# markkurossi/mpc

Hardware: AMD Instinct MI355X
Metric: AND-gates/sec (garble+eval), AES-128 circuit batch (higher is better)
Workload: dtype u32 (AES T-table / 128-bit label XOR, integer); 1 GPU; aes_128.circ 36663 gates / 6400 AND, batch=1024 instances per GPU, 32-byte garbling key; instances_per_gpu=1024, levels=308, launches_per_garble=1, schedule=fused-flat, hash_phases=89, lds_live_labels=1053, graph=True, outputs_ok=True, device_memory=gc_dev_alloc / gc_dev_upload (C ABI); no torch in the process, gathers=0

## Files before the change

### include/gcengine.h

```cpp
#ifndef GCENGINE_H
#define GCENGINE_H

#include <stddef.h>
#include <stdint.h>

#ifdef __cplusplus
extern "C" {
#endif

typedef struct gc_label { uint64_t d0, d1; } gc_label;
typedef struct gc_wire { gc_label l0, l1; } gc_wire;
typedef struct gc_gate {
    uint32_t in0, in1, out;
    uint8_t op;
    uint8_t pad_[3];
    uint32_t level;
} gc_gate;

enum {
    GC_XOR = 0, GC_XNOR = 1, GC_AND = 2, GC_OR = 3, GC_INV = 4
};

enum {
    GC_OK = 0,
// ... 23 lines not shown
    uint32_t n_xor, n_xnor, n_and, n_or, n_inv;
    uint32_t nslots;
    uint32_t n_steps;
    uint32_t n_hash_phases;
    uint32_t n_fused_steps;
    uint32_t n_lds_slots;
    uint32_t n_flat_slots;
    uint32_t n_flat_outs;
    uint32_t n_flat_terms;
    uint32_t n_flat_steps;
    uint32_t n_flat_units;
} gc_plan_info;

gc_plan *gc_plan_create(const gc_gate *gates, uint32_t ngates, uint32_t nwires, uint32_t ninputs,
                        uint32_t noutputs, int *status);
gc_plan *gc_plan_create_chain(const gc_gate *const *gates, const uint32_t *ngates, const uint32_t *nwires, const uint32_t *nin,
                              const uint32_t *nout, const uint32_t *const *wiring, uint32_t nsteps, int *status);
void gc_plan_free(gc_plan *);
int gc_plan_get_info(const gc_plan *, gc_plan_info *out);
int gc_plan_simulate(const gc_plan *, const uint8_t *in_bits, uint8_t *out_bits);
int gc_plan_describe(const gc_plan *, uint32_t *level_of_gate, uint32_t *tweak_of_gate,
                     uint32_t *row_of_gate, uint32_t *slot_of_gate);
int gc_plan_fingerprint(const gc_plan *, uint64_t *fp);

typedef struct gc_ctx gc_ctx;
typedef struct gc_circ gc_circ;

int gc_device_count(void);
gc_ctx *gc_ctx_create(int device, int *status);
void gc_ctx_destroy(gc_ctx *);
int gc_ctx_sync(gc_ctx *);
int gc_ctx_coop_stats(gc_ctx *, int *state, uint64_t *timeouts);
int gc_ctx_pci_bus_id(gc_ctx *, char *buf, size_t len);
void *gc_ctx_stream(gc_ctx *);

typedef struct gc_graph gc_graph;
int gc_ctx_capture_begin(gc_ctx *);
int gc_ctx_capture_end(gc_ctx *, gc_graph **out);
int gc_graph_launch(gc_graph *);
void gc_graph_free(gc_graph *);

gc_circ *gc_circ_load(gc_ctx *, const gc_gate *gates, uint32_t ngates, uint32_t nwires,
                      uint32_t ninputs, uint32_t noutputs, int *status);
void gc_circ_free(gc_circ *);
const gc_plan *gc_circ_plan(const gc_circ *);
int gc_circ_set_schedule(gc_circ *, int schedule);
// ... 313 lines not shown
```

### mpc_amd/csrc/aes_device.h

```cpp
#pragma once

#include <hip/hip_runtime.h>

#include <cstdint>

namespace gc {

constexpr int kTeWords = 4 * 256;

__device__ __forceinline__ uint32_t rotr32(uint32_t v, uint32_t n) { return __builtin_amdgcn_alignbit(v, v, n); }

__device__ __forceinline__ void load_te_tables(uint32_t *te, const uint32_t *__restrict__ g_te0) {
    for (uint32_t i = threadIdx.x; i < 256; i += blockDim.x) {
        uint32_t t = g_te0[i];
        te[i] = t;
        te[256 + i] = rotr32(t, 8);
        te[512 + i] = rotr32(t, 16);
        te[768 + i] = rotr32(t, 24);
    }
}

template <int NR, int N>
__device__ __forceinline__ void aes_encrypt_n(uint32_t (&s)[N][4], const uint32_t *__restrict__ rk,
                                              const uint32_t *te) {
// ... 78 lines not shown
        s[k][0] = GC_LAST(a0, a1, a2, a3) ^ rk[4 * NR + 0];
        s[k][1] = GC_LAST(a1, a2, a3, a0) ^ rk[4 * NR + 1];
        s[k][2] = GC_LAST(a2, a3, a0, a1) ^ rk[4 * NR + 2];
        s[k][3] = GC_LAST(a3, a0, a1, a2) ^ rk[4 * NR + 3];
#undef GC_LAST
#undef GC_SB
    }
}

constexpr int kTeDualBytes = 256 * 256;

__device__ __forceinline__ void te_dual_check(const uint32_t *te);

__device__ __forceinline__ void load_te_dual(uint32_t *te, const uint32_t *__restrict__ g_te0) {
    te_dual_check(te);
    const uint32_t c = threadIdx.x & 31;
    for (uint32_t x = threadIdx.x >> 5; x < 256; x += blockDim.x >> 5) {
        const uint32_t t = g_te0[x];
        te[x * 64 + c] = t;
        te[x * 64 + 32 + c] = rotr32(t, 16);
    }
}

#define GC_PERM_SEL(k) (0x0c0c0000u | ((4u + (k)) << 8))

using lds_u32 = __attribute__((address_space(3))) const uint32_t;

__device__ __forceinline__ void te_dual_check(const uint32_t *te) {
    if ((uint32_t)(uintptr_t)te != 0u) __builtin_trap();
}

__device__ __forceinline__ uint32_t te_dual(uint32_t word, uint32_t sel, uint32_t lane_off) {
    const uint32_t addr = __builtin_amdgcn_perm(word, lane_off, sel);
    return *(lds_u32 *)(uintptr_t)addr;
}

__device__ __forceinline__ uint32_t xor3(uint32_t a, uint32_t b, uint32_t c) {
    return __builtin_amdgcn_bitop3_b32(a, b, c, 0x96);
}

__device__ __forceinline__ void te_round_addrs(const uint32_t (&a)[4], uint32_t lo0, uint32_t lo2, uint32_t (&ad)[16]) {
    const uint32_t sel0 = GC_PERM_SEL(0), sel1 = GC_PERM_SEL(1), sel2 = GC_PERM_SEL(2), sel3 = GC_PERM_SEL(3);
#pragma unroll
    for (int c = 0; c < 4; c++) {
        ad[4 * c + 0] = __builtin_amdgcn_perm(a[c], lo0, sel3);
        ad[4 * c + 1] = __builtin_amdgcn_perm(a[(c + 2) & 3], lo2, sel1);
// ... 136 lines not shown
            __builtin_amdgcn_sched_barrier(0);
#pragma unroll
            for (int k = 0; k < N; k++)
#pragma unroll
                for (int i = 0; i < 16; i++) t[k][i] = *(lds_u32 *)(uintptr_t)ad[k][i];
            __builtin_amdgcn_sched_barrier(0);
            te_final_combine<NR, N, FEED>(t, rk, fin, s);
        }
    }
}

template <int NR>
__device__ __forceinline__ void load_round_keys(uint32_t (&rk)[4 * (NR + 1)], const uint32_t *__restrict__ g_rk) {
#pragma unroll
    for (int i = 0; i < 4 * (NR + 1); i++) rk[i] = __builtin_amdgcn_readfirstlane(g_rk[i]);
}

template <int NR, int NS>
__device__ __forceinline__ void load_round_keys_split(uint32_t (&rk)[4 * (NR + 1)], const uint32_t *__restrict__ g_rk,
                                                      uint32_t vz) {
#pragma unroll
    for (int i = 0; i < 4 * (NR + 1); i++)
        rk[i] = i < NS ? (uint32_t)__builtin_amdgcn_readfirstlane(g_rk[i]) : g_rk[i + vz];
}

template <int NR, int N>
__device__ __forceinline__ void hash_dual_n(const uint32_t (&k)[N][4], uint4 (&out)[N],
                                            const uint32_t (&rk)[4 * (NR + 1)], const uint32_t *te, uint32_t lo0) {
    uint32_t s[N][4];
#pragma unroll
    for (int i = 0; i < N; i++) {
        s[i][0] = k[i][0];
        s[i][1] = k[i][1];
        s[i][2] = k[i][2];
        s[i][3] = k[i][3];
    }
    aes_encrypt_dual<NR, N, 1>(s, rk, te, lo0);
#pragma unroll
    for (int i = 0; i < N; i++) out[i] = make_uint4(s[i][1], s[i][0], s[i][3], s[i][2]);
}

template <int NR>
__device__ __forceinline__ uint4 hash_dual(const uint32_t (&k)[4], const uint32_t (&rk)[4 * (NR + 1)],
                                           const uint32_t *te, uint32_t lo0) {
    uint32_t s[1][4] = {{k[0], k[1], k[2], k[3]}};
    aes_encrypt_dual<NR, 1, 1>(s, rk, te, lo0);
// ... 143 lines not shown
```

### mpc_amd/csrc/engine.cpp

```cpp
#include "engine.h"

#include <algorithm>
#include <atomic>
#include <chrono>
#include <cstdlib>
#include <cstdio>
#include <cstring>
#include <new>
#include <stdexcept>

namespace gc {

thread_local char tls_error[512] = "";

void set_error(const char *what, hipError_t e) {
    std::snprintf(tls_error, sizeof tls_error, "%s: %s (%d)", what, hipGetErrorString(e), (int)e);
    (void)hipGetLastError();
}

int on_exception() noexcept {
    try {
        throw;
    } catch (const std::bad_alloc &) {
        std::snprintf(tls_error, sizeof tls_error, "host allocation failed (std::bad_alloc)");
// ... 775 lines not shown
static int run_levels(gc_batch *b, bool eval, const uint4 *T, const uint4 *rnd = nullptr) {
    hipStream_t s = b->circ->ctx->stream;
    const Plan &p = b->circ->plan.p;
    if (b->schedule == 1 && b->g.lds_wires && want_flat(b)) {
        FusedFlatArgs f{};
        f.prog = b->circ->d_fl_prog;
        f.units = b->circ->d_fl_units;
        f.hgslot = b->circ->d_fl_hgslot;
        f.ogslot = b->circ->d_fl_ogslot;
        f.in_lds = b->circ->d_fl_in_lds;
        f.nunits = (uint32_t)p.fl_units.size();
        f.ninputs = p.info.ninputs;
        f.nls = p.n_flat_slots;
        f.ustride = p.fl_unit_stride;
        f.W = b->d_W;
        f.R = b->d_R;
        f.T = const_cast<uint4 *>(T);
        f.rk = b->d_rk;
        f.te0 = b->circ->ctx->d_te0;
        f.rounds = b->rounds;
        f.prof = b->d_prof;
        f.rnd = rnd;
        f.has_or = p.info.n_or != 0;
        GC_HIP(launch_fused_flat(eval, f, b->g, s));
        b->last_launches = f.nunits ? 1 : 0;
        b->have_all_wires = false;
        return GC_OK;
    }
    if (b->schedule == 1 && b->g.lds_wires) {
        FusedLdsArgs f{};
        f.descs = b->circ->d_fdescs;
        f.gslot = b->circ->d_fgslot;
        f.steps = b->circ->d_fsteps;
        f.in_lds = b->circ->d_in_lds;
        f.nsteps = (uint32_t)p.fsteps.size();
        f.chunks = b->circ->d_fchunks;
        f.nchunks = (uint32_t)p.fchunks.size();
        f.ninputs = p.info.ninputs;
        f.nls = p.n_lds_slots;
        f.W = b->d_W;
        f.R = b->d_R;
        f.T = const_cast<uint4 *>(T);
        f.rk = b->d_rk;
        f.te0 = b->circ->ctx->d_te0;
        f.rounds = b->rounds;
        f.store_all = b->store_all;
// ... 659 lines not shown
}
bool gc_circ_flat_job(gc_circ *c, gc::FlatJob *j, size_t *lds_bytes, bool *has_or) {
    if (!c || !j) return false;
    circ_ensure_flat(c);
    const Plan &p = c->plan.p;
    if (p.n_flat_slots == 0xffffffffu || p.fl_units.empty() || p.info.slab_rows >= (1u << 22) || !c->d_fl_prog) return false;
    const size_t need = fused_flat_bytes(p.n_flat_slots, 0, p.fl_unit_stride);
    if (need > (size_t)160 * 1024) return false;
    *j = FlatJob{};
    j->prog = (const uint4 *)c->d_fl_prog;
    j->units = c->d_fl_units;
    j->hgslot = c->d_fl_hgslot;
    j->ogslot = c->d_fl_ogslot;
    j->in_lds = c->d_fl_in_lds;
    j->nunits = (uint32_t)p.fl_units.size();
    j->ninputs = p.info.ninputs;
    j->ti_log2 = 0;
    j->zslot = p.n_flat_slots - 1;
    j->ustride = p.fl_unit_stride;
    j->w_tile = p.info.nslots;
    j->t_tile = std::max<uint32_t>(p.info.slab_rows, 1);
    j->te0 = c->ctx->d_te0;
    j->batch = 1;
    if (lds_bytes) *lds_bytes = need;
    if (has_or) *has_or = p.info.n_or != 0;
    return true;
}

void gc_circ_release_batch(gc_circ *c, gc_batch *b) {
    if (c && b) pool_put(c, b);
}

int gc_pass_dev(gc_circ *c, bool eval, const uint8_t *key, size_t keylen, const gc_label *r, const void *d_store,
                const uint32_t *d_in_idx, const uint32_t *d_out_idx, const gc_label *slab_host, size_t slab_rows,
                gc_batch **bout, const gc::StoreXchg *d_xchg) {
    if (!c || !bout || !d_store || (!eval && !r)) return GC_E_ARG;
    gc_batch *b = *bout;
    *bout = nullptr;
    const Plan &p = c->plan.p;
    if (b && (b->circ != c || b->g.batch != 1)) return GC_E_ARG;
    if (eval && (slab_rows != p.info.slab_rows || (!slab_host && slab_rows && !b))) {
        if (b) pool_put(c, b);
        return GC_E_ROWS;
    }
    int rc = GC_OK;
    if (!b) b = pool_get(c, 1, &rc);
// ... 234 lines not shown
```

### mpc_amd/csrc/fused_flat_kernels.hip

```cpp
#include "aes_device.h"
#include "kernels.h"

namespace gc {

namespace {

constexpr int TF = 1024;

constexpr int DPP_XOR1 = 0xB1;
constexpr int DPP_XOR2 = 0x4E;
constexpr int DPP_XOR3 = 0x1B;
constexpr int DPP_BC0 = 0x00;
constexpr int DPP_BC2 = 0xAA;
constexpr int DPP_PAIR0 = 0xA0;

template <int CTRL>
__device__ __forceinline__ uint32_t dpp32(uint32_t v) {
    return (uint32_t)__builtin_amdgcn_mov_dpp((int)v, CTRL, 0xf, 0xf, true);
}
template <int CTRL>
__device__ __forceinline__ uint4 dpp128(uint4 v) {
    return make_uint4(dpp32<CTRL>(v.x), dpp32<CTRL>(v.y), dpp32<CTRL>(v.z), dpp32<CTRL>(v.w));
}

// ... 320 lines not shown
    const uint64_t *q = (const uint64_t *)p;
    const uint64_t lo = __hip_atomic_load(q, __ATOMIC_RELAXED, __HIP_MEMORY_SCOPE_AGENT);
    const uint64_t hi = __hip_atomic_load(q + 1, __ATOMIC_RELAXED, __HIP_MEMORY_SCOPE_AGENT);
    return make_uint4((uint32_t)lo, (uint32_t)(lo >> 32), (uint32_t)hi, (uint32_t)(hi >> 32));
}
__device__ __forceinline__ void store_put(uint4 *p, const uint4 &v) {
    uint64_t *q = (uint64_t *)p;
    __hip_atomic_store(q, (uint64_t)v.x | ((uint64_t)v.y << 32), __ATOMIC_RELAXED, __HIP_MEMORY_SCOPE_AGENT);
    __hip_atomic_store(q + 1, (uint64_t)v.z | ((uint64_t)v.w << 32), __ATOMIC_RELAXED, __HIP_MEMORY_SCOPE_AGENT);
}

constexpr uint32_t kDepSpins = 1u << 22;
__device__ __forceinline__ uint32_t fresh_u32(const uint32_t *p) { return __hip_atomic_load(p, __ATOMIC_RELAXED, __HIP_MEMORY_SCOPE_AGENT); }
__device__ __forceinline__ void df_wait_reached(const uint32_t *p, uint32_t want, uint32_t *host_err) {
    for (uint32_t spins = 0; (int32_t)(__hip_atomic_load(p, __ATOMIC_RELAXED, __HIP_MEMORY_SCOPE_AGENT) - want) < 0;) {
        __builtin_amdgcn_s_sleep(8);
        if (++spins > kDepSpins) {
            if (host_err) __hip_atomic_fetch_max(host_err, 3u, __ATOMIC_RELAXED, __HIP_MEMORY_SCOPE_SYSTEM);
            break;
        }
    }
}

#define GC_FL_PROLOGUE(LOAD_R)                                                                               \
    const uint32_t tile = MULTI ? 0u : blockIdx.x;                                                           \
    extern __shared__ uint4 smem[];                                                                          \
    uint32_t *te = (uint32_t *)smem;                                                                         \
    const uint32_t ti_log2 = a.ti_log2, TI = 1u << ti_log2, tim = TI - 1;                                    \
    uint4 *stage = smem + kStageOff;                                                                         \
    const uint32_t ustride = a.ustride;                                                                      \
    uint4 *rl = smem + kStageOff + 2 * ustride;                                                              \
    uint4 *wl = rl + TI;                                                                                     \
     \
    const bool first_job = !MULTI || a.pad2_ == 0;                                                           \
    if (first_job) load_te_dual(te, a.te0);                                                                  \
    uint32_t rkr[4 * (NR + 1)];                                                                              \
    uint32_t vz;                                                                                             \
    asm volatile("v_mov_b32 %0, 0" : "=v"(vz));                                                              \
    load_round_keys_split<NR, (4 * (NR + 1) > 32 ? 4 * (NR + 1) - 32 : 4 * (NR + 1))>(rkr, a.rk, vz);        \
    fold_last_round_key<NR>(rkr);               \
    if (first_job && threadIdx.x < 4 * (NR + 1)) {  \
        uint32_t kv = a.rk[threadIdx.x];                                                                     \
        if (threadIdx.x >= 4 * NR) kv ^= a.rk[threadIdx.x - 4 * NR];                                         \
        ((uint32_t *)smem)[kKeyTab / 4 + threadIdx.x] = kv;                                                  \
    }                                                                                                        \
    uint4 *Wt = a.W + (size_t)tile * a.w_tile;                                                               \
    if (threadIdx.x < TI) wl[(a.zslot << ti_log2) + threadIdx.x] = make_uint4(0, 0, 0, 0);                   \
    if (LOAD_R && a.rnd) {                                                                                   \
         \
         \
        for (uint32_t i = threadIdx.x; i < ((a.ninputs + 1) << ti_log2); i += TF) {                          \
            const uint32_t j = i >> ti_log2, inst = i & tim, gi = tile * TI + inst;                          \
            uint4 v = make_uint4(0, 0, 0, 0);                                                                \
            if (gi < a.batch) {                                                                              \
                const uint4 raw = a.rnd[(size_t)gi * (a.ninputs + 1) + j];                                   \
                v = make_uint4(__builtin_bswap32(raw.y), __builtin_bswap32(raw.x), __builtin_bswap32(raw.w), \
                               __builtin_bswap32(raw.z));                                                    \
            }                                                                                                \
            if (j == 0) {                                                                                    \
                v.y |= 0x80000000u;                                                        \
                rl[inst] = v;                                                                                \
                a.Rout[(size_t)tile * TI + inst] = v;                                                        \
            } else {                                                                                         \
                const uint32_t ls = a.in_lds[j - 1];                                                         \
                Wt[((j - 1) << ti_log2) + inst] = v;                                                         \
                if (ls != 0xffffu) wl[(ls << ti_log2) + inst] = v;                                           \
            }                                                                                                \
        }                                                                                                    \
    } else {                                                                                                 \
        if (LOAD_R && threadIdx.x < TI) rl[threadIdx.x] = a.R[(size_t)tile * TI + threadIdx.x];              \
        for (uint32_t i = threadIdx.x; i < (a.ninputs << ti_log2); i += TF) {                                \
            const uint32_t w = i >> ti_log2, ls = a.in_lds[w];                                               \
            if constexpr (MULTI) {            \
                const DfBlock *dfb = LOAD_R ? (const DfBlock *)a.prof : nullptr;  \
                const uint32_t sidx = dfb ? fresh_u32(a.in_idx + w) : a.in_idx[w];                           \
                if (dfb) df_wait_reached(dfb->ver + sidx, fresh_u32((const uint32_t *)(dfb + 1) + w), dfb->host_err); \
                const uint4 v = store_get(a.store + sidx);                                                   \
                Wt[i] = v;                                                                                   \
                if (ls != 0xffffu) wl[(ls << ti_log2) + (i & tim)] = v;                                      \
                if (dfb) {  \
                    asm volatile("s_waitcnt vmcnt(0)" ::: "memory");                                         \
                    __hip_atomic_fetch_add(dfb->rd + sidx, 1u, __ATOMIC_RELAXED, __HIP_MEMORY_SCOPE_AGENT);  \
                }                                                                                            \
            } else if (ls != 0xffffu) {                                                                      \
                wl[(ls << ti_log2) + (i & tim)] = Wt[i];                                                     \
            }                                                                                                \
        }                                                                                                    \
    }                                                                                                        \
    FUnit u = uniform_unit(load_unit(a.units, 0, vz));                                             \
     \
     \
    FUnit un = load_unit(a.units, 1, vz);                                                          \
    if (threadIdx.x < u.n16) stage[threadIdx.x] = a.prog[u.off16 + threadIdx.x];                             \
     \
     \
    uint4 pre_cur = a.prog[un.off16 + threadIdx.x];                                                          \
    __syncthreads();                                                                                         \
    const uint32_t lo = te_lane_off();                                                                       \
    const uint32_t wave_base = __builtin_amdgcn_readfirstlane(threadIdx.x & ~63u);                           \
    uint64_t pacc[8] = {0, 0, 0, 0, 0, 0, 0, 0}, plast = 0;                                                  \
    if constexpr (PROF) plast = __builtin_amdgcn_s_memtime();

}

template <int NR, bool PROF, bool HAS_OR, bool MULTI>
__device__ __forceinline__ void garble_flat_body(const FlArgs &a) {
    GC_FL_PROLOGUE(true)
    uint4 *Tt = a.T + (size_t)tile * a.t_tile;
    for (uint32_t ui = 0; ui < a.nunits; ui++) {
        const uint4 *buf = stage + (ui & 1u) * ustride;
        const uint32_t nh = u.n_and + u.n_or + u.n_inv;
        GC_FPROF(0)
        const uint32_t e_hash = hlanes<2, 2, 1>(u, ti_log2);
        if (nh && u.n_or == 0 && e_hash <= kNarrowLanes) {
            garble_hash_narrow<NR, PROF>(buf, u, a, ti_log2, tim, wl, rl, Tt, Wt, lo, HashSplit{0, e_hash, 0}, pacc, &plast);
        } else if (nh) {
            const HashSplit hs = split_hash_lanes(e_hash, u.n_or != 0, kTailMaxGarble);
            const uint32_t e_all = hs.wide_end;
        for (uint32_t t0 = 0; t0 + wave_base < e_all; t0 += TF) {
// ... 380 lines not shown
hipError_t launch_fused_flat(bool eval, const FusedFlatArgs &f, const BatchGeom &g, hipStream_t s) {
    FlArgs a{};
    a.prog = (const uint4 *)f.prog;
    a.units = f.units;
    a.hgslot = f.hgslot;
    a.ogslot = f.ogslot;
    a.in_lds = f.in_lds;
    a.nunits = f.nunits;
    a.ninputs = f.ninputs;
    a.ti_log2 = g.ti_log2;
    a.zslot = f.nls - 1;
    a.ustride = f.ustride;
    a.w_tile = g.lw.tile_stride;
    a.t_tile = g.lt.tile_stride;
    a.W = f.W;
    a.R = f.R;
    a.T = f.T;
    a.rk = f.rk;
    a.te0 = f.te0;
    a.prof = f.prof;
    a.rnd = eval ? nullptr : f.rnd;
    a.Rout = const_cast<uint4 *>(f.R);
    a.batch = g.batch;
    if (a.nunits == 0) return hipSuccess;
    const size_t lds = fused_flat_bytes(f.nls, g.ti_log2, f.ustride);
#define GC_M3(KERN, NR)                                                                      \
    (f.prof ? (f.has_or ? launch_fl(KERN<NR, true, true>, a, g.ntiles, lds, s)               \
                        : launch_fl(KERN<NR, true, false>, a, g.ntiles, lds, s))             \
            : f.has_or ? launch_fl(KERN<NR, false, true>, a, g.ntiles, lds, s)              \
                       : launch_fl(KERN<NR, false, false>, a, g.ntiles, lds, s))
#define GC_M2(KERN) (f.rounds == 10 ? GC_M3(KERN, 10) : f.rounds == 12 ? GC_M3(KERN, 12) : GC_M3(KERN, 14))
    return eval ? GC_M2(k_eval_flat) : GC_M2(k_garble_flat);
#undef GC_M2
#undef GC_M3
}

template <typename K>
static hipError_t launch_jobs(K kern, const FlatJob *jobs, const uint32_t *first, uint32_t *sync, uint32_t nunits, size_t lds,
                              hipStream_t s) {
    hipError_t e = hipFuncSetAttribute((const void *)kern, hipFuncAttributeMaxDynamicSharedMemorySize, (int)lds);
    if (e != hipSuccess) return e;
    hipLaunchKernelGGL(kern, dim3(nunits), dim3(TF), lds, s, jobs, first, sync);
    return hipGetLastError();
}

template <typename K>
// ... 36 lines not shown
```

### mpc_amd/csrc/kernels.h

```cpp
#pragma once

#include <hip/hip_runtime.h>

#include <cstdint>

#include "co_multi_table.h"
#include "co_table.h"
#include "p256.h"
#include "plan.h"
#include "vole_mod.h"

namespace gc {

struct Layout {
    uint32_t ti_log2;
    uint32_t ti_mask;
    size_t row_stride;
    size_t tile_stride;
#if defined(__HIPCC__)
    __host__ __device__
#endif
    size_t at(size_t row, uint32_t inst) const {
        return (size_t)(inst >> ti_log2) * tile_stride + row * row_stride + (inst & ti_mask);
    }
// ... 83 lines not shown
    int rounds;
    bool store_all;
    uint64_t *prof;
};
size_t fused_lds_bytes(uint32_t nls, uint32_t ti_log2);
hipError_t launch_fused_lds(bool eval, const FusedLdsArgs &a, const BatchGeom &g, hipStream_t s);

struct FusedFlatArgs {
    const uint32_t *prog;
    const FUnit *units;
    const uint32_t *hgslot, *ogslot;
    const uint16_t *in_lds;
    uint32_t nunits, ninputs, nls;
    uint32_t ustride;
    uint4 *W;
    const uint4 *R;
    uint4 *T;
    const uint32_t *rk;
    const uint32_t *te0;
    int rounds;
    uint64_t *prof;
    const uint4 *rnd;
    bool has_or;
};
size_t fused_flat_bytes(uint32_t nls, uint32_t ti_log2, uint32_t ustride);
hipError_t launch_fused_flat(bool eval, const FusedFlatArgs &a, const BatchGeom &g, hipStream_t s);

struct FlatJob {
    const uint4 *prog;
    const FUnit *units;
    const uint32_t *hgslot, *ogslot;
    const uint16_t *in_lds;
    uint32_t nunits, ninputs, ti_log2, zslot;
    uint32_t ustride;
    size_t w_tile, t_tile;
    uint4 *W;
    const uint4 *R;
    uint4 *T;
    const uint32_t *rk;
    const uint32_t *te0;
    uint64_t *prof;
    const uint4 *rnd;
    uint4 *Rout;
    uint32_t batch;
    uint32_t pad_;
    uint4 *store;
    const uint32_t *in_idx;
    const uint32_t *out_slots;
    const uint32_t *out_idx;
    uint32_t nout, pad2_;
};
constexpr uint32_t kSyncHead = 4;
struct DfBlock {
    uint32_t *ver, *rd;
    uint32_t *host_err;
    uint32_t nin, nout;
    uint32_t pad_[2];
};
static_assert(sizeof(DfBlock) == 40 || sizeof(DfBlock) == 48, "DfBlock layout");
constexpr uint32_t kPoolRing = 8192;
constexpr uint32_t kPoolGroups = 8192;
struct PoolEntry {
    const FlatJob *rec;
    uint32_t more, group;
};
struct PoolCtl {
    uint32_t head, tail;
    uint32_t done_total, pad_;
    uint32_t *host_err;
    uint32_t persist, stop;
    uint32_t done[kPoolGroups];
    PoolEntry ring[kPoolRing];
};
hipError_t launch_fused_flat_pool(int rounds, PoolCtl *ctl, uint32_t nworkers, size_t lds_bytes, hipStream_t s);
// ... 140 lines not shown
```

### mpc_amd/csrc/plan.cpp

```cpp
#include "plan.h"

#include <algorithm>
#include <chrono>
#include <cstdio>
#include <cstdlib>
#include <map>
#include <numeric>

namespace gc {

namespace {
struct PlanLaps {
    bool on = std::getenv("GC_TRACE") != nullptr;
    std::chrono::steady_clock::time_point t = std::chrono::steady_clock::now();
    void lap(const char *what) {
        if (!on) return;
        const auto n = std::chrono::steady_clock::now();
        std::fprintf(stderr, "[gc trace] plan: %-28s %8.3f ms\n", what, std::chrono::duration<double, std::milli>(n - t).count());
        t = n;
    }
};
}

static inline int op_class(uint8_t op) {
// ... 813 lines not shown

int gc_plan_fingerprint(const gc_plan *pl, uint64_t *fp) try {
    if (!pl || !fp) return GC_E_ARG;
    const gc::Plan &p = pl->p;
    uint64_t h = 14695981039346656037ull;
    auto mix = [&h](const void *data, size_t n) {
        const uint8_t *b = (const uint8_t *)data;
        for (size_t i = 0; i < n; i++) h = (h ^ b[i]) * 1099511628211ull;
        h = (h ^ (uint64_t)n) * 1099511628211ull;
    };
    auto vec = [&mix](const auto &v) { mix(v.data(), v.size() * sizeof(v[0])); };
    vec(p.descs), vec(p.levels), vec(p.out_slots);
    vec(p.fdescs), vec(p.fgslot), vec(p.fsteps), vec(p.fchunks), vec(p.in_lds);
    vec(p.fl_prog), vec(p.fl_units), vec(p.fl_hgslot), vec(p.fl_ogslot), vec(p.fl_in_lds);
    const uint32_t tail[8] = {p.n_flat_slots, p.n_flat_outs, p.n_flat_terms, p.n_flat_steps, p.flat_late ? 1u : 0u,
                              p.fl_unit_stride, p.fl_max_parts, p.n_lds_slots};
    mix(tail, sizeof tail);
    *fp = h;
    return GC_OK;
} catch (...) {
    return gc::on_exception();
}

int gc_plan_describe(const gc_plan *pl, uint32_t *level_of_gate, uint32_t *tweak_of_gate, uint32_t *row_of_gate,
                     uint32_t *slot_of_gate) try {
    if (!pl) return GC_E_ARG;
    const gc::Plan &p = pl->p;
    if (level_of_gate) std::copy(p.level_of_gate.begin(), p.level_of_gate.end(), level_of_gate);
    if (tweak_of_gate) std::copy(p.tweak_of_gate.begin(), p.tweak_of_gate.end(), tweak_of_gate);
    if (row_of_gate) std::copy(p.row_of_gate.begin(), p.row_of_gate.end(), row_of_gate);
    if (slot_of_gate) std::copy(p.slot_of_gate.begin(), p.slot_of_gate.end(), slot_of_gate);
    return GC_OK;
} catch (...) {
    return gc::on_exception();
}

}
```

### mpc_amd/csrc/plan.h

```cpp
#pragma once

#include <cstdint>
#include <vector>

#include "../../include/gcengine.h"

namespace gc {

int on_exception() noexcept;

struct GateDesc {
    uint32_t in0;
    uint32_t in1;
    uint32_t tweak;
    uint32_t row_op;
};
static_assert(sizeof(GateDesc) == 16, "GateDesc must be 16 bytes");

constexpr uint32_t kOpShift = 29;
constexpr uint32_t kRowMask = (1u << kOpShift) - 1;

struct Step {
    uint32_t first;
    uint32_t count;
// ... 25 lines not shown
    uint16_t flags;
    uint16_t n;
    uint16_t pad_;
};
static_assert(sizeof(XOut) == 24, "XOut must be 24 bytes");
constexpr uint16_t kXoStore = 1;
constexpr uint16_t kXoRpar = 2;
constexpr uint16_t kXoJoin2 = 4;
constexpr uint16_t kXoJoin4 = 8;
constexpr uint16_t kXoPart = 16;
constexpr uint32_t kUHash = 256, kUOuts = 448;
constexpr uint32_t kUnit16 = kUHash + kUOuts * 24 / 16;
struct FUnit {
    uint32_t off16, n16;
    uint32_t n_and, n_or, n_inv;
    uint32_t nout;
    uint32_t outs_off16;
    uint32_t xparts;
    uint32_t hfirst, ofirst;
    uint32_t pad_[2];
};
static_assert(sizeof(FUnit) == 48, "FUnit must be 48 bytes");

struct Plan {
    gc_plan_info info{};
    std::vector<uint32_t> level_of_gate, tweak_of_gate, row_of_gate , slot_of_gate;
    std::vector<GateDesc> descs;
    std::vector<uint32_t> gate_of_desc;
    std::vector<Step> levels;
    std::vector<uint32_t> slot_of_wire;
    std::vector<uint32_t> out_slots;

    std::vector<FDesc> fdescs;
    std::vector<uint32_t> fgslot;
    std::vector<Step> fsteps;
    std::vector<Chunk> fchunks;
    std::vector<uint32_t> fl_prog;
    std::vector<FUnit> fl_units;
    std::vector<uint32_t> fl_hgslot, fl_ogslot;
    std::vector<uint16_t> fl_in_lds;
    uint32_t n_flat_slots = 0xffffffffu;
    uint32_t n_flat_outs = 0, n_flat_terms = 0, n_flat_steps = 0;
    bool flat_late = false;
    uint32_t fl_unit_stride = 0;
    uint32_t fl_max_parts = 1;
    std::vector<uint16_t> in_lds;
// ... 24 lines not shown
```

### mpc_amd/engine.py

```python
import ctypes as C
import os
import subprocess

import numpy as np

from .circuit import GATE, LABEL, WIRE

HERE = os.path.dirname(os.path.abspath(__file__))
CSRC = os.path.join(HERE, "csrc")
LIB_PATH = os.environ.get("GC_LIB") or os.path.join(CSRC, "libgcengine.so")
HEADER = os.path.join(os.path.dirname(HERE), "include", "gcengine.h")

ABI_VERSION = 2
GC_OK, GC_E_KEYSIZE, GC_E_RAND, GC_E_GATE, GC_E_ROWS, GC_E_ARG, GC_E_HIP, GC_E_NOMEM, GC_E_WIRE, GC_E_POINT = (
    0, -1, -2, -3, -4, -5, -6, -7, -8, -9)


class EngineError(RuntimeError):

    def __init__(self, code, what=""):
        self.code = code
        msg = lib().gc_strerror(code).decode() if _lib is not None else "status %d" % code
        detail = lib().gc_last_error().decode() if _lib is not None and code in (GC_E_HIP, GC_E_NOMEM) else ""
        super().__init__("%s%s%s" % (what + ": " if what else "", msg, " [" + detail + "]" if detail else ""))
# ... 25 lines not shown

def lib():
    global _lib
    if _lib is not None:
        return _lib
    if not os.path.exists(LIB_PATH):
        raise ImportError("%s is missing: run `python -c 'import __graft_entry__ as g; g.build()'` "
                          "(the HIP extension is the product; there is no CPU fallback)" % LIB_PATH)
    os.environ.setdefault("GPU_MAX_HW_QUEUES", "8")
    L = C.CDLL(LIB_PATH)
    vp, u32, sz, i32 = C.c_void_p, C.c_uint32, C.c_size_t, C.c_int
    ip = C.POINTER(C.c_int)
    sigs = {
        "gc_strerror": (C.c_char_p, [i32]),
        "gc_last_error": (C.c_char_p, []),
        "gc_abi_version": (i32, []),
        "gc_plan_create": (vp, [vp, u32, u32, u32, u32, ip]),
        "gc_plan_create_chain": (vp, [vp, vp, vp, vp, vp, vp, u32, ip]),
        "gc_plan_free": (None, [vp]),
        "gc_plan_get_info": (i32, [vp, C.POINTER(PlanInfo)]),
        "gc_plan_simulate": (i32, [vp, vp, vp]),
        "gc_plan_describe": (i32, [vp, vp, vp, vp, vp]),
        "gc_plan_fingerprint": (i32, [vp, vp]),
        "gc_device_count": (i32, []),
        "gc_ctx_create": (vp, [i32, ip]),
        "gc_ctx_destroy": (None, [vp]),
        "gc_ctx_sync": (i32, [vp]),
        "gc_ctx_stream": (vp, [vp]),
        "gc_circ_load": (vp, [vp, vp, u32, u32, u32, u32, ip]),
        "gc_circ_free": (None, [vp]),
        "gc_circ_plan": (vp, [vp]),
        "gc_circ_set_schedule": (i32, [vp, i32]),
        "gc_garble": (i32, [vp, vp, sz, vp, sz, u32, vp, vp, vp, vp]),
        "gc_eval": (i32, [vp, vp, sz, u32, vp, vp, vp, sz, vp]),
        "gc_garble_labels": (i32, [vp, vp, sz, vp, vp, vp, vp]),
        "gc_stream_create": (vp, [vp, vp, sz, vp, sz, vp, u32, ip]),
        "gc_stream_free": (None, [vp]),
        "gc_stream_get_wire": (i32, [vp, u32, vp]),
        "gc_stream_garble": (i32, [vp, vp, u32, u32, vp, u32, vp, u32, vp, sz, C.POINTER(C.c_size_t)]),
        "gc_stream_garble_begin": (i32, [vp, vp, u32, u32, vp, u32, vp, u32]),
        "gc_stream_garble_finish": (i32, [vp, vp, sz, C.POINTER(C.c_size_t)]),
        "gc_stream_garble_flush": (i32, [vp]),
        "gc_stream_intern": (i32, [vp, vp, u32, u32, u32, u32, C.POINTER(C.c_uint32)]),
        "gc_stream_garble_begin_h": (i32, [vp, u32, vp, vp]),
        "gc_stream_release": (i32, [vp, u32]),
        "gc_stream_garble_finish_view": (i32, [vp, C.POINTER(C.c_void_p), C.POINTER(C.c_size_t)]),
# ... 268 lines not shown
        gp, wp = (C.c_void_p * n)(), (C.c_void_p * n)()
        ng, nw, ni, no = (np.zeros(n, np.uint32) for _ in range(4))
        for k, (gates, nwires, nin, nout, wiring) in enumerate(steps):
            g = np.ascontiguousarray(gates, dtype=GATE)
            w = np.full(nin, 0xFFFFFFFF, np.uint32) if wiring is None else np.ascontiguousarray(wiring, dtype=np.uint32)
            assert len(w) == nin
            keep += [g, w]
            gp[k], wp[k] = g.ctypes.data, w.ctypes.data
            ng[k], nw[k], ni[k], no[k] = len(g), nwires, nin, nout
        st = C.c_int(0)
        self = cls.__new__(cls)
        self.h = L.gc_plan_create_chain(gp, _p(ng), _p(nw), _p(ni), _p(no), wp, n, C.byref(st))
        if not self.h:
            raise EngineError(st.value, "gc_plan_create_chain")
        self._describe(int(ng.sum()))
        self.gate_base = np.concatenate([[0], np.cumsum(ng)]).astype(np.uint32)
        return self

    def fingerprint(self):
        fp = C.c_uint64(0)
        _check(lib().gc_plan_fingerprint(self.h, C.byref(fp)), "gc_plan_fingerprint")
        return "%016x" % fp.value

    def simulate(self, in_bits):
        b = np.ascontiguousarray(in_bits, dtype=np.uint8)
        assert len(b) == self.info.ninputs
        out = np.zeros(max(self.info.noutputs, 1), np.uint8)
        _check(lib().gc_plan_simulate(self.h, _p(b) if len(b) else None, _p(out)), "gc_plan_simulate")
        return out[: self.info.noutputs]

    def __del__(self):
        if getattr(self, "h", None) and _lib is not None:
            _lib.gc_plan_free(self.h)
            self.h = None




class Context:
    def __init__(self, device=0):
        st = C.c_int(0)
        self.h = lib().gc_ctx_create(device, C.byref(st))
        if not self.h:
            raise EngineError(st.value, "gc_ctx_create(%d)" % device)
        self.device = device

# ... 1427 lines not shown
```

Before: 6.783 billion AND-gates/s.

## Overlap fused-flat prologue loads by issuing global reads before LDS commits

Restructures the fused-flat kernel prologue into issue and commit phases. T-table rows, round keys, the first program images, input labels and R are all loaded into registers up front and written to LDS afterwards, so their global latencies overlap instead of serialising. For single-job launches the first two unit offsets are passed as kernel arguments, taken from a new host-side flat_head helper, so the dependent unit-descriptor load leaves the critical path. The change costs extra VGPR pressure in the prologue and makes the MULTI and dataflow paths more complex, which raises correctness risk.

New measurement: 6.805 billion AND-gates/s (median of 6 runs). About the same (+0.3%).

```diff
diff --git a/include/gcengine.h b/include/gcengine.h
--- a/include/gcengine.h
+++ b/include/gcengine.h
@@ -69,6 +69,7 @@
 int gc_plan_describe(const gc_plan *, uint32_t *level_of_gate, uint32_t *tweak_of_gate,
                      uint32_t *row_of_gate, uint32_t *slot_of_gate);
 int gc_plan_fingerprint(const gc_plan *, uint64_t *fp);
+int gc_plan_flat_head(const gc_plan *, uint32_t head[3], uint32_t *off16, uint32_t *n16);
 
 typedef struct gc_ctx gc_ctx;
 typedef struct gc_circ gc_circ;
diff --git a/mpc_amd/csrc/aes_device.h b/mpc_amd/csrc/aes_device.h
--- a/mpc_amd/csrc/aes_device.h
+++ b/mpc_amd/csrc/aes_device.h
@@ -124,6 +124,31 @@
     }
 }
 
+template <int THREADS>
+struct TeDualRows {
+    static_assert(THREADS % 32 == 0 && (256 * 32) % THREADS == 0, "whole rows per pass of the workgroup");
+    static constexpr int kRows = 256 * 32 / THREADS;
+    uint32_t t[kRows];
+};
+template <int THREADS>
+__device__ __forceinline__ TeDualRows<THREADS> te_dual_issue(const uint32_t *__restrict__ g_te0) {
+    TeDualRows<THREADS> r;
+#pragma unroll
+    for (int k = 0; k < TeDualRows<THREADS>::kRows; k++) r.t[k] = g_te0[(threadIdx.x >> 5) + k * (THREADS / 32)];
+    return r;
+}
+template <int THREADS>
+__device__ __forceinline__ void te_dual_commit(uint32_t *te, const TeDualRows<THREADS> &r) {
+    te_dual_check(te);
+    const uint32_t c = threadIdx.x & 31;
+#pragma unroll
+    for (int k = 0; k < TeDualRows<THREADS>::kRows; k++) {
+        const uint32_t x = (threadIdx.x >> 5) + k * (THREADS / 32);
+        te[x * 64 + c] = r.t[k];
+        te[x * 64 + 32 + c] = rotr32(r.t[k], 16);
+    }
+}
+
 #define GC_PERM_SEL(k) (0x0c0c0000u | ((4u + (k)) << 8))
 
 using lds_u32 = __attribute__((address_space(3))) const uint32_t;
@@ -306,6 +331,17 @@
 #pragma unroll
     for (int i = 0; i < 4 * (NR + 1); i++)
         rk[i] = i < NS ? (uint32_t)__builtin_amdgcn_readfirstlane(g_rk[i]) : g_rk[i + vz];
+}
+
+template <int NR>
+__device__ __forceinline__ void round_keys_issue(uint32_t (&rk)[4 * (NR + 1)], const uint32_t *__restrict__ g_rk, uint32_t vz) {
+#pragma unroll
+    for (int i = 0; i < 4 * (NR + 1); i++) rk[i] = g_rk[i + vz];
+}
+template <int NR, int NS>
+__device__ __forceinline__ void round_keys_split_finish(uint32_t (&rk)[4 * (NR + 1)]) {
+#pragma unroll
+    for (int i = 0; i < NS; i++) rk[i] = (uint32_t)__builtin_amdgcn_readfirstlane(rk[i]);
 }
 
 template <int NR, int N>
diff --git a/mpc_amd/csrc/engine.cpp b/mpc_amd/csrc/engine.cpp
--- a/mpc_amd/csrc/engine.cpp
+++ b/mpc_amd/csrc/engine.cpp
@@ -821,6 +821,7 @@
         f.prof = b->d_prof;
         f.rnd = rnd;
         f.has_or = p.info.n_or != 0;
+        f.head = flat_head(p.fl_units.data(), p.fl_units.size());
         GC_HIP(launch_fused_flat(eval, f, b->g, s));
         b->last_launches = f.nunits ? 1 : 0;
         b->have_all_wires = false;
@@ -1526,6 +1527,8 @@
     j->t_tile = std::max<uint32_t>(p.info.slab_rows, 1);
     j->te0 = c->ctx->d_te0;
     j->batch = 1;
+    const FlatHead h = flat_head(p.fl_units.data(), p.fl_units.size());
+    j->off16_0 = h.off16_0, j->n16_0 = h.n16_0, j->off16_1 = h.off16_1;
     if (lds_bytes) *lds_bytes = need;
     if (has_or) *has_or = p.info.n_or != 0;
     return true;
diff --git a/mpc_amd/csrc/fused_flat_kernels.hip b/mpc_amd/csrc/fused_flat_kernels.hip
--- a/mpc_amd/csrc/fused_flat_kernels.hip
+++ b/mpc_amd/csrc/fused_flat_kernels.hip
@@ -366,6 +366,11 @@
     }
 }
 
+struct FlIn {
+    uint4 v;
+    uint32_t ls;
+};
+
 #define GC_FL_PROLOGUE(LOAD_R)                                                                               \
     const uint32_t tile = MULTI ? 0u : blockIdx.x;                                                           \
     extern __shared__ uint4 smem[];                                                                          \
@@ -377,68 +382,159 @@
     uint4 *wl = rl + TI;                                                                                     \
      \
     const bool first_job = !MULTI || a.pad2_ == 0;                                                           \
-    if (first_job) load_te_dual(te, a.te0);                                                                  \
     uint32_t rkr[4 * (NR + 1)];                                                                              \
     uint32_t vz;                                                                                             \
     asm volatile("v_mov_b32 %0, 0" : "=v"(vz));                                                              \
-    load_round_keys_split<NR, (4 * (NR + 1) > 32 ? 4 * (NR + 1) - 32 : 4 * (NR + 1))>(rkr, a.rk, vz);        \
-    fold_last_round_key<NR>(rkr);               \
-    if (first_job && threadIdx.x < 4 * (NR + 1)) {  \
-        uint32_t kv = a.rk[threadIdx.x];                                                                     \
-        if (threadIdx.x >= 4 * NR) kv ^= a.rk[threadIdx.x - 4 * NR];                                         \
-        ((uint32_t *)smem)[kKeyTab / 4 + threadIdx.x] = kv;                                                  \
-    }                                                                                                        \
     uint4 *Wt = a.W + (size_t)tile * a.w_tile;                                                               \
-    if (threadIdx.x < TI) wl[(a.zslot << ti_log2) + threadIdx.x] = make_uint4(0, 0, 0, 0);                   \
-    if (LOAD_R && a.rnd) {                                                                                   \
-         \
-         \
-        for (uint32_t i = threadIdx.x; i < ((a.ninputs + 1) << ti_log2); i += TF) {                          \
-            const uint32_t j = i >> ti_log2, inst = i & tim, gi = tile * TI + inst;                          \
-            uint4 v = make_uint4(0, 0, 0, 0);                                                                \
-            if (gi < a.batch) {                                                                              \
-                const uint4 raw = a.rnd[(size_t)gi * (a.ninputs + 1) + j];                                   \
-                v = make_uint4(__builtin_bswap32(raw.y), __builtin_bswap32(raw.x), __builtin_bswap32(raw.w), \
-                               __builtin_bswap32(raw.z));                                                    \
+    const bool from_rnd = LOAD_R && !MULTI && a.rnd;    \
+     \
+     \
+    const DfBlock *dfb = (MULTI && LOAD_R && !from_rnd) ? (const DfBlock *)a.prof : nullptr;                 \
+    const bool via_store = MULTI && !from_rnd;      \
+     \
+     \
+    const uint32_t n_in = from_rnd ? (a.ninputs + 1) << ti_log2 : a.ninputs << ti_log2;                      \
+     \
+     \
+     \
+     \
+    auto in_issue = [&](uint32_t i) {                                                                        \
+        FlIn x{make_uint4(0, 0, 0, 0), 0xffffu};                                                             \
+        if constexpr (MULTI) {  \
+            if (i < n_in) {              \
+                x.ls = a.in_lds[i >> ti_log2];                                                               \
+                x.v.x = a.in_idx[i >> ti_log2];                                                              \
             }                                                                                                \
+        } else {                                                                                             \
+            const uint32_t ic = i < n_in ? i : 0u;                                                           \
+            uint32_t w = ic >> ti_log2;               \
+            const uint4 *src = Wt;                                                                           \
+            size_t at = ic;                                                                                  \
+            if (from_rnd) {                                                                                  \
+                const uint32_t gi = tile * TI + (ic & tim);                                                  \
+                src = a.rnd;                                                                                 \
+                at = (size_t)(gi < a.batch ? gi : a.batch - 1) * (a.ninputs + 1) + w;                        \
+                w = w ? w - 1 : 0u;                                                                          \
+            }                                                                                                \
+            x.v = src[at];                                                                                   \
+            x.ls = (a.ninputs ? a.in_lds : (const uint16_t *)a.units)[w];                                    \
+        }                                                                                                    \
+        (void)via_store;                                                                                     \
+        return x;                                                                                            \
+    };                                                                                                       \
+    auto in_commit = [&](uint32_t i, const FlIn &x) {                                                        \
+        if (i >= n_in) return;                                                                               \
+        const uint32_t inst = i & tim;                                                                       \
+        if (from_rnd) {                                                                                      \
+            const uint32_t j = i >> ti_log2;                                                                 \
+            uint4 v = make_uint4(__builtin_bswap32(x.v.y), __builtin_bswap32(x.v.x), __builtin_bswap32(x.v.w), \
+                                 __builtin_bswap32(x.v.z));                                                  \
+            if (tile * TI + inst >= a.batch) v = make_uint4(0, 0, 0, 0);                                     \
             if (j == 0) {                                                                                    \
                 v.y |= 0x80000000u;                                                        \
                 rl[inst] = v;                                                                                \
                 a.Rout[(size_t)tile * TI + inst] = v;                                                        \
             } else {                                                                                         \
-                const uint32_t ls = a.in_lds[j - 1];                                                         \
                 Wt[((j - 1) << ti_log2) + inst] = v;                                                         \
-                if (ls != 0xffffu) wl[(ls << ti_log2) + inst] = v;                                           \
+                if (x.ls != 0xffffu) wl[(x.ls << ti_log2) + inst] = v;                                       \
             }                                                                                                \
+        } else {                                                                                             \
+            if constexpr (MULTI) Wt[i] = x.v;                                                                \
+            if (x.ls != 0xffffu) wl[(x.ls << ti_log2) + inst] = x.v;  \
         }                                                                                                    \
+    };                                                                                                       \
+                                                                                    \
+    FlIn in0{make_uint4(0, 0, 0, 0), 0xffffu}, in1 = in0;                                                    \
+    if constexpr (MULTI) {                                                                                   \
+        if (!dfb) in0 = in_issue(threadIdx.x);  \
+    }                                                                                                        \
+    const FUnit u_v = load_unit(a.units, 0, vz);                                                             \
+     \
+     \
+    FUnit un = load_unit(a.units, 1, vz);                                                                    \
+     \
+     \
+    uint4 img0, pre_cur;                                                                                     \
+    if constexpr (!MULTI) {                                                                                  \
+        img0 = a.prog[a.off16_0 + threadIdx.x];                                                              \
+        pre_cur = a.prog[a.off16_1 + threadIdx.x];                                                           \
+    }                                                                                                        \
+    round_keys_issue<NR>(rkr, a.rk, vz);                                                                     \
+     \
+    const bool key_lane = first_job && threadIdx.x < 4 * (NR + 1);                                           \
+    const uint32_t kl = threadIdx.x < 4 * (NR + 1) ? threadIdx.x : 0u;                                       \
+    const bool r_lane = LOAD_R && !from_rnd && threadIdx.x < TI;                                             \
+    uint32_t kv = 0, kv0 = 0;                                                                                \
+    uint4 r_v = make_uint4(0, 0, 0, 0);                                                                      \
+    if constexpr (MULTI) {                                                                                   \
+        if (key_lane) {                                                                                      \
+            kv = a.rk[threadIdx.x];                                                                          \
+            if (threadIdx.x >= 4 * NR) kv0 = a.rk[threadIdx.x - 4 * NR];                                     \
+        }                                                                                                    \
+        if (r_lane) r_v = a.R[threadIdx.x];                                                                  \
     } else {                                                                                                 \
-        if (LOAD_R && threadIdx.x < TI) rl[threadIdx.x] = a.R[(size_t)tile * TI + threadIdx.x];              \
-        for (uint32_t i = threadIdx.x; i < (a.ninputs << ti_log2); i += TF) {                                \
-            const uint32_t w = i >> ti_log2, ls = a.in_lds[w];                                               \
-            if constexpr (MULTI) {            \
-                const DfBlock *dfb = LOAD_R ? (const DfBlock *)a.prof : nullptr;  \
-                const uint32_t sidx = dfb ? fresh_u32(a.in_idx + w) : a.in_idx[w];                           \
-                if (dfb) df_wait_reached(dfb->ver + sidx, fresh_u32((const uint32_t *)(dfb + 1) + w), dfb->host_err); \
+        kv = a.rk[kl], kv0 = a.rk[kl >= 4 * NR ? kl - 4 * NR : 0u];                                          \
+        if (threadIdx.x < 4 * NR) kv0 = 0;                                                                   \
+        if constexpr (LOAD_R) r_v = (from_rnd ? a.rnd : a.R + (size_t)tile * TI)[threadIdx.x < TI ? threadIdx.x : 0u]; \
+    }                                                                                                        \
+    FUnit u;                                                                                                 \
+    if constexpr (MULTI) {                                                                                   \
+         \
+         \
+         \
+        u = uniform_unit(u_v);                                                                               \
+        round_keys_split_finish<NR, (4 * (NR + 1) > 32 ? 4 * (NR + 1) - 32 : 4 * (NR + 1))>(rkr);            \
+        __builtin_amdgcn_sched_barrier(0);                                                                   \
+        img0 = a.prog[u.off16 + threadIdx.x];                                                                \
+        pre_cur = a.prog[un.off16 + threadIdx.x];                                                            \
+        if (via_store && !dfb && threadIdx.x < n_in) in0.v = store_get(a.store + in0.v.x);                   \
+    } else {                                                                                                 \
+        in0 = in_issue(threadIdx.x);                                                                         \
+        in1 = in_issue(threadIdx.x + TF);                \
+    }                                                                                                        \
+    TeDualRows<TF> te_v{};                                                                                   \
+    if (first_job) te_v = te_dual_issue<TF>(a.te0);                                                          \
+    __builtin_amdgcn_sched_barrier(0);                                                                       \
+                                                          \
+    if (threadIdx.x < TI) wl[(a.zslot << ti_log2) + threadIdx.x] = make_uint4(0, 0, 0, 0);                   \
+    if constexpr (!MULTI) {                                                                                  \
+        u = uniform_unit(u_v);                                                                               \
+        round_keys_split_finish<NR, (4 * (NR + 1) > 32 ? 4 * (NR + 1) - 32 : 4 * (NR + 1))>(rkr);            \
+    }                                                                                                        \
+    if (threadIdx.x < (MULTI ? u.n16 : a.n16_0)) stage[threadIdx.x] = img0;                                  \
+    fold_last_round_key<NR>(rkr);                \
+    if (key_lane) ((uint32_t *)smem)[kKeyTab / 4 + threadIdx.x] = kv ^ kv0;                                  \
+    if (r_lane) rl[threadIdx.x] = r_v;                                                                       \
+    if (!dfb) in_commit(threadIdx.x, in0);                             \
+    if constexpr (!MULTI) in0 = in_issue(threadIdx.x + 2 * TF);  \
+    if (first_job) te_dual_commit<TF>(te, te_v);                                                             \
+    if (dfb) {                                                                                               \
+        if constexpr (MULTI) {                                                                               \
+            for (uint32_t i = threadIdx.x; i < n_in; i += TF) {                                              \
+                const uint32_t w = i >> ti_log2, ls = a.in_lds[w];                                           \
+                const uint32_t sidx = fresh_u32(a.in_idx + w);                 \
+                df_wait_reached(dfb->ver + sidx, fresh_u32((const uint32_t *)(dfb + 1) + w), dfb->host_err); \
                 const uint4 v = store_get(a.store + sidx);                                                   \
                 Wt[i] = v;                                                                                   \
                 if (ls != 0xffffu) wl[(ls << ti_log2) + (i & tim)] = v;                                      \
-                if (dfb) {  \
-                    asm volatile("s_waitcnt vmcnt(0)" ::: "memory");                                         \
-                    __hip_atomic_fetch_add(dfb->rd + sidx, 1u, __ATOMIC_RELAXED, __HIP_MEMORY_SCOPE_AGENT);  \
-                }                                                                                            \
-            } else if (ls != 0xffffu) {                                                                      \
-                wl[(ls << ti_log2) + (i & tim)] = Wt[i];                                                     \
+                 \
+                asm volatile("s_waitcnt vmcnt(0)" ::: "memory");                                             \
+                __hip_atomic_fetch_add(dfb->rd + sidx, 1u, __ATOMIC_RELAXED, __HIP_MEMORY_SCOPE_AGENT);      \
             }                                                                                                \
         }                                                                                                    \
+    } else if constexpr (MULTI) {  \
+        for (uint32_t i = threadIdx.x + TF; i < n_in; i += TF) {                                             \
+            FlIn x = in_issue(i);                                                                            \
+            if (via_store) x.v = store_get(a.store + x.v.x);                                                 \
+            in_commit(i, x);                                                                                 \
+        }                                                                                                    \
+    } else {                                                                                                 \
+        for (uint32_t i = threadIdx.x + TF; i < n_in; i += TF) {                                             \
+            in_commit(i, in1);                                                                               \
+            in1 = in0;                                                                                       \
+            in0 = in_issue(i + 2 * TF);                                                                      \
+        }                                                                                                    \
     }                                                                                                        \
-    FUnit u = uniform_unit(load_unit(a.units, 0, vz));                                             \
-     \
-     \
-    FUnit un = load_unit(a.units, 1, vz);                                                          \
-    if (threadIdx.x < u.n16) stage[threadIdx.x] = a.prog[u.off16 + threadIdx.x];                             \
-     \
-     \
-    uint4 pre_cur = a.prog[un.off16 + threadIdx.x];                                                          \
     __syncthreads();                                                                                         \
     const uint32_t lo = te_lane_off();                                                                       \
     const uint32_t wave_base = __builtin_amdgcn_readfirstlane(threadIdx.x & ~63u);                           \
@@ -865,6 +961,7 @@
     a.rnd = eval ? nullptr : f.rnd;
     a.Rout = const_cast<uint4 *>(f.R);
     a.batch = g.batch;
+    a.off16_0 = f.head.off16_0, a.n16_0 = f.head.n16_0, a.off16_1 = f.head.off16_1;
     if (a.nunits == 0) return hipSuccess;
     const size_t lds = fused_flat_bytes(f.nls, g.ti_log2, f.ustride);
 #define GC_M3(KERN, NR)                                                                      \
diff --git a/mpc_amd/csrc/kernels.h b/mpc_amd/csrc/kernels.h
--- a/mpc_amd/csrc/kernels.h
+++ b/mpc_amd/csrc/kernels.h
@@ -129,6 +129,7 @@
     uint64_t *prof;
     const uint4 *rnd;
     bool has_or;
+    FlatHead head;
 };
 size_t fused_flat_bytes(uint32_t nls, uint32_t ti_log2, uint32_t ustride);
 hipError_t launch_fused_flat(bool eval, const FusedFlatArgs &a, const BatchGeom &g, hipStream_t s);
@@ -156,7 +157,9 @@
     const uint32_t *out_slots;
     const uint32_t *out_idx;
     uint32_t nout, pad2_;
-};
+    uint32_t off16_0, n16_0, off16_1, pad3_;
+};
+static_assert(sizeof(FlatJob) % 8 == 0, "FlatJob: records lie back to back in an upload region, pointers first");
 constexpr uint32_t kSyncHead = 4;
 struct DfBlock {
     uint32_t *ver, *rd;
diff --git a/mpc_amd/csrc/plan.cpp b/mpc_amd/csrc/plan.cpp
--- a/mpc_amd/csrc/plan.cpp
+++ b/mpc_amd/csrc/plan.cpp
@@ -859,6 +859,21 @@
     return gc::on_exception();
 }
 
+int gc_plan_flat_head(const gc_plan *pl, uint32_t head[3], uint32_t *off16, uint32_t *n16) try {
+    if (!pl || !head) return GC_E_ARG;
+    const gc::Plan &p = pl->p;
+    if (p.n_flat_slots == 0xffffffffu || p.fl_units.empty()) return GC_E_ARG;
+    const gc::FlatHead h = gc::flat_head(p.fl_units.data(), p.fl_units.size());
+    head[0] = h.off16_0, head[1] = h.n16_0, head[2] = h.off16_1;
+    for (size_t i = 0; i < p.fl_units.size(); i++) {
+        if (off16) off16[i] = p.fl_units[i].off16;
+        if (n16) n16[i] = p.fl_units[i].n16;
+    }
+    return GC_OK;
+} catch (...) {
+    return gc::on_exception();
+}
+
 int gc_plan_describe(const gc_plan *pl, uint32_t *level_of_gate, uint32_t *tweak_of_gate, uint32_t *row_of_gate,
                      uint32_t *slot_of_gate) try {
     if (!pl) return GC_E_ARG;
diff --git a/mpc_amd/csrc/plan.h b/mpc_amd/csrc/plan.h
--- a/mpc_amd/csrc/plan.h
+++ b/mpc_amd/csrc/plan.h
@@ -71,6 +71,13 @@
 };
 static_assert(sizeof(FUnit) == 48, "FUnit must be 48 bytes");
 
+struct FlatHead {
+    uint32_t off16_0, n16_0, off16_1;
+};
+inline FlatHead flat_head(const FUnit *units, size_t nunits) {
+    return FlatHead{nunits > 0 ? units[0].off16 : 0u, nunits > 0 ? units[0].n16 : 0u, nunits > 1 ? units[1].off16 : 0u};
+}
+
 struct Plan {
     gc_plan_info info{};
     std::vector<uint32_t> level_of_gate, tweak_of_gate, row_of_gate , slot_of_gate;
diff --git a/mpc_amd/engine.py b/mpc_amd/engine.py
--- a/mpc_amd/engine.py
+++ b/mpc_amd/engine.py
@@ -71,6 +71,7 @@
         "gc_plan_simulate": (i32, [vp, vp, vp]),
         "gc_plan_describe": (i32, [vp, vp, vp, vp, vp]),
         "gc_plan_fingerprint": (i32, [vp, vp]),
+        "gc_plan_flat_head": (i32, [vp, vp, vp, vp]),
         "gc_device_count": (i32, []),
         "gc_ctx_create": (vp, [i32, ip]),
         "gc_ctx_destroy": (None, [vp]),
@@ -385,6 +386,12 @@
         _check(lib().gc_plan_fingerprint(self.h, C.byref(fp)), "gc_plan_fingerprint")
         return "%016x" % fp.value
 
+    def flat_head(self):
+        n = self.info.n_flat_units
+        head, off16, n16 = np.zeros(3, np.uint32), np.zeros(n, np.uint32), np.zeros(n, np.uint32)
+        _check(lib().gc_plan_flat_head(self.h, _p(head), _p(off16), _p(n16)), "gc_plan_flat_head")
+        return head, off16, n16
+
     def simulate(self, in_bits):
         b = np.ascontiguousarray(in_bits, dtype=np.uint8)
         assert len(b) == self.info.ninputs
```
